# ssmiler/tfhe_fbs_map

Measured on AMD Instinct MI355X. Metric: functional bootstraps/sec (batched), N=1024, higher is better.
Workload: dtype f64 (exact integer arithmetic mod a 46-bit prime via FMA; residues in 64-bit words)

## Files before the change

### tfhe_fbs_map_amd/_native.py

```python
from __future__ import annotations

import ctypes as C
import operator
import os
import weakref

import numpy as np

_HERE = os.path.dirname(os.path.abspath(__file__))
LIB_PATH = os.environ.get("FBS_LIB") or os.path.join(_HERE, "libfbsexec.so")

from .security import MODULUS, MODULUS_BITS, sigma_min
from . import _client_native, _public_native
from ._client_native import GAUSSIAN_SAMPLER_GRADE, RANDOMNESS_GRADE, SAMPLERS, ClientContext, FbsError, Params, _Params, _c, _ptr, gpu_library_missing


class _Layout(C.Structure):
    _fields_ = [(f, C.c_uint32) for f in ("n_slots", "n_levels", "max_width", "max_sources", "n_bootstrap", "n_keyswitch",
                                          "n_inputs", "n_outputs", "n_rotations", "row_words")]


class _ProgramDesc(C.Structure):
    _fields_ = [("n_inputs", C.c_uint32), ("n_instr", C.c_uint32), ("n_terms", C.c_uint32),
                ("n_outputs", C.c_uint32),
# ... 751 lines not shown
        self._check(lib.fbs_refresh_compact_dev(self._h, d_words or None, count, self.default_compact_bits if bits is None else int(bits),
                                                d_cts or None, stream or None))

    def decrypt_compact_dev(self, d_words, count, d_msgs, bits=None, stream=0):
        self._check(lib.fbs_decrypt_compact_dev(self._h, d_words or None, count, self.default_compact_bits if bits is None else int(bits),
                                                d_msgs or None, stream or None))

    def _import_gadget_key(self, noun, t, gamma, bodies):
        bodies = _c(bodies, np.uint64).reshape(-1)
        if 1 <= int(t) <= 31 and bodies.size != self._gadget_key_sizes(noun, t)[0]:
            raise ValueError(f"{noun}_bodies has {bodies.size} words, the parameter set needs {self._gadget_key_sizes(noun, t)[0]}")
        self._check(getattr(lib, f"fbs_import_{noun}_key")(self._h, int(t), int(gamma), _ptr(bodies)))

    def import_packing_key(self, t_p, gamma_p, bodies):
        self._import_gadget_key("packing", t_p, gamma_p, bodies)

    def fold_keygen(self, t_f, gamma_f):
        self._check(lib.fbs_fold_keygen(self._h, int(t_f), int(gamma_f)))

    def fold_key_sizes(self, t_f=0):
        return self._gadget_key_sizes("fold", t_f)

    def export_fold_key(self, full=False):
        return self._export_gadget_key("fold", self.params.k * self.params.N, full)

    def import_fold_key(self, t_f, gamma_f, bodies):
        self._import_gadget_key("fold", t_f, gamma_f, bodies)

    def fold_dev(self, d_cts, count, d_glwe, stream=0):
        self._check(lib.fbs_fold_dev(self._h, d_cts or None, int(count), d_glwe or None, stream or None))

    def fold_mapped_dev(self, d_cts, n_src, d_map, count, d_glwe, stream=0):
        self._check(lib.fbs_fold_mapped_dev(self._h, d_cts or None, int(n_src), d_map or None, int(count), d_glwe or None, stream or None))

    def lookup_dev(self, d_tables, n_tables, d_table_of, d_cts_index, count, d_cts_out, stream=0):
        self._check(lib.fbs_lookup_dev(self._h, d_tables or None, int(n_tables), d_table_of or None, d_cts_index or None, int(count),
                                       d_cts_out or None, stream or None))

    def lookup_compact_dev(self, d_tables, n_tables, d_table_of, d_words, count, d_cts_out, bits=None, stream=0):
        self._check(lib.fbs_lookup_compact_dev(self._h, d_tables or None, int(n_tables), d_table_of or None, d_words or None, int(count),
                                               self.default_compact_bits if bits is None else int(bits), d_cts_out or None, stream or None))

    def rotate_dev(self, d_tables, n_tables, d_table_of, d_cts_index, count, d_glwe_out, negate=False, stream=0):
        self._check(lib.fbs_rotate_dev(self._h, d_tables or None, int(n_tables), d_table_of or None, d_cts_index or None, int(count),
                                       ROTATE_NEGATE if negate else 0, d_glwe_out or None, stream or None))

    def rotate_compact_dev(self, d_tables, n_tables, d_table_of, d_words, count, d_glwe_out, bits=None, negate=False, stream=0):
        self._check(lib.fbs_rotate_compact_dev(self._h, d_tables or None, int(n_tables), d_table_of or None, d_words or None, int(count),
                                               self.default_compact_bits if bits is None else int(bits), ROTATE_NEGATE if negate else 0,
                                               d_glwe_out or None, stream or None))

    def glwe_add_dev(self, d_dst, n_dst, dst_of, d_src, stream=0):
        dst_of = _c(dst_of, np.uint32).reshape(-1)
        self._check(lib.fbs_glwe_add_dev(self._h, d_dst or None, int(n_dst), _ptr(dst_of), d_src or None, dst_of.size, stream or None))

    def debug_fold_front_dev(self, d_cts, count, cols, tg, d_fields, stream=0):
        self._check(lib.fbs_debug_fold_front_dev(self._h, d_cts or None, int(count), int(cols), int(tg), d_fields or None, stream or None))

    def fold(self, cts):
        import torch
        cts = _c(cts, np.uint64).reshape(-1, self.params.ct_words)
        count, prm = cts.shape[0], self.params
        words = -(-count // prm.N) * (prm.k + 1) * prm.N
        dev = f"cuda:{self.device}"
        d_c = torch.from_numpy(cts.view(np.int64)).to(dev) if count else torch.zeros(1, dtype=torch.int64, device=dev)
        d_w = torch.zeros(max(2, words), dtype=torch.int64, device=dev)
        torch.cuda.synchronize(d_w.device)
        self.fold_dev(d_c.data_ptr(), count, d_w.data_ptr())
        self.sync()
        return d_w[:words].cpu().numpy().view(np.uint64)

    def pack_dev(self, d_cts, count, d_words, bits, stream=0):
        self._check(lib.fbs_pack_dev(self._h, d_cts or None, int(count), int(bits), d_words or None, stream or None))

    def debug_pack_fields_dev(self, d_fields, count, d_words, bits, stream=0):
        self._check(lib.fbs_debug_pack_fields_dev(self._h, d_fields or None, int(count), int(bits), d_words or None, stream or None))

    def pack(self, cts, bits):
        import torch
        cts = _c(cts, np.uint64).reshape(-1, self.params.ct_words)
        count = cts.shape[0]
        d_c = torch.from_numpy(cts.view(np.int64)).to("cuda:%d" % self.device)
        d_w = torch.zeros(max(1, self.packed_words(count, bits)), dtype=torch.int64, device=d_c.device)
        torch.cuda.synchronize(d_c.device)
        self.pack_dev(d_c.data_ptr(), count, d_w.data_ptr(), bits)
        self.sync()
        return d_w[:self.packed_words(count, bits)].cpu().numpy().view(np.uint64)

    def bootstrap_batch(self, tvset, cts, table_ids=None):
        cts = _c(cts, np.uint64)
        count = cts.size // self.params.ct_words
        ids = None if table_ids is None else _c(table_ids, np.uint32)
        out = np.empty_like(cts)
        self._check(lib.fbs_bootstrap_batch(self._h, tvset._h, _ptr(cts), _ptr(ids), count, _ptr(out)))
        return out

    def encrypt_dev(self, d_msgs, count, d_cts, nonce0=None, stream=0):
        if nonce0 is None:
            first = C.c_uint64()
            self._check(lib.fbs_encrypt_fresh_dev(self._h, d_msgs or None, count, d_cts or None, C.byref(first), stream or None))
            return first.value
        self._check(lib.fbs_encrypt_dev(self._h, d_msgs or None, count, int(nonce0), d_cts or None, stream or None))
        return int(nonce0)

    def decrypt_dev(self, d_cts, count, d_msgs, stream=0):
        self._check(lib.fbs_decrypt_dev(self._h, d_cts or None, count, d_msgs or None, stream or None))

    def bootstrap_batch_dev(self, tvset, d_in, d_table_ids, count, d_out, stream=0):
        self._check(lib.fbs_bootstrap_batch_dev(self._h, tvset._h, d_in, d_table_ids or None, count, d_out,
                                                stream or None))

    def lincomb_dev(self, d_wires, T, dst, term_off, srcs, coefs, consts, stream=0):
        dst, term_off, srcs = _c(dst, np.uint32), _c(term_off, np.uint32), _c(srcs, np.uint32)
        coefs, consts = _c(coefs, np.int64), _c(consts, np.int64)
        self._check(lib.fbs_lincomb_dev(self._h, d_wires, T, len(dst), _ptr(dst), _ptr(term_off), _ptr(srcs),
                                        _ptr(coefs), _ptr(consts), stream or None))

    def bootstrap_wires_dev(self, tvset, d_wires, T, src, dst, table_ids, s_begin, s_end, stream=0):
        src, dst, table_ids = _c(src, np.uint32), _c(dst, np.uint32), _c(table_ids, np.uint32)
        self._check(lib.fbs_bootstrap_wires_dev(self._h, tvset._h, d_wires, T, len(src), _ptr(src), _ptr(dst),
                                                _ptr(table_ids), s_begin, s_end, stream or None))

    def profile(self, on=True):
        self._check(lib.fbs_profile_enable(self._h, int(on)))

    def profile_read(self, reset=True):
        ms = (C.c_double * 3)()
        cnt = (C.c_uint64 * 3)()
        self._check(lib.fbs_profile_read(self._h, C.byref(ms), C.byref(cnt), int(reset)))
        names = ("keyswitch", "blind_rotate", "lincomb")
        return {n: dict(ms=ms[i], launches=int(cnt[i]), kernel=lib.fbs_profile_kernel(self._h, i).decode())
                for i, n in enumerate(names)}

    def profile_kernels(self):
        need = C.c_size_t()
        self._check(lib.fbs_profile_kernels(self._h, None, 0, C.byref(need)))
        buf = C.create_string_buffer(need.value)
        self._check(lib.fbs_profile_kernels(self._h, buf, need.value, None))
        out = {}
        for line in buf.value.decode().splitlines():
            kind, name, launches, ms = line.split("\t")
            out[name] = dict(kind=("keyswitch", "blind_rotate", "lincomb")[int(kind)], launches=int(launches), ms=float(ms))
        return out

    def sync(self, stream=0):
        self._check(lib.fbs_sync(self._h, stream or None))

    def debug_polymul(self, a, b):
        a, b = _c(a, np.uint64), _c(b, np.uint64)
        c = np.empty_like(a)
        self._check(lib.fbs_debug_polymul(self._h, _ptr(a), _ptr(b), _ptr(c)))
        return c

    DEBUG_FIELD_OPS = ("fp_mulmod", "fp_mulmod_exact", "fp_center", "fp_canon", "fp_canon_near", "fp_u64_round_trip")

    def debug_field(self, op, x, w=None):
        x = _c(x, np.int64)
        w = None if w is None else _c(w, np.int64)
        out = np.empty_like(x)
        self._check(lib.fbs_debug_field(self._h, self.DEBUG_FIELD_OPS.index(op), _ptr(x), _ptr(w), x.size, _ptr(out)))
        return out

    def debug_gauss_dev(self, words, sigma):
        import torch
        words = _c(words, np.uint64).reshape(-1, 6)
        dev = torch.device("cuda", self.device)
        d_words = torch.from_numpy(words.view(np.int64)).to(dev)
        d_out = torch.empty(words.shape[0], dtype=torch.int64, device=dev)
        self._check(lib.fbs_debug_gauss_dev(self._h, d_words.data_ptr(), words.shape[0], int(sigma), d_out.data_ptr(), None))
        self.sync()
        return d_out.cpu().numpy()

    def debug_transform(self, variant, values):
        values = _c(values, np.int64).reshape(-1, 1 << self.params.log_n_poly)
        out = np.empty_like(values)
        self._check(lib.fbs_debug_transform(self._h, variant.encode(), _ptr(values), _ptr(out), values.shape[0]))
        return out
```

### tfhe_fbs_map_amd/csrc/fbs_blind_rotate.hip

```cpp
#include <hip/hip_runtime.h>

#include <algorithm>
#include <type_traits>
#include <utility>

#include "fbs_blind_rotate.hpp"

namespace fbs {

template <int LOGN, int LL>
__global__ __launch_bounds__(1 << LL) void k_polymul(const uint64_t *a, const uint64_t *b, uint64_t *c, const double *tw_fwd,
                                                     const double *tw_inv, double n_inv) {
    using W = typename NttFor<LOGN, LL>::type;
    __shared__ double lds[2 * W::N];
    const uint32_t t = threadIdx.x;
    typename W::Xchg xc{lds, 0};
    double x[W::E], y[W::E];
#pragma unroll
    for (int m = 0; m < W::E; m++) {
        x[m] = fp_from_u64(a[W::template index_of<0>(t, m)]);
        y[m] = fp_from_u64(b[W::template index_of<0>(t, m)]);
    }
    W::forward(x, xc, t, Twiddles(tw_fwd + W::LANE_TABLE_OFFSET, tw_fwd));
    W::forward(y, xc, t, Twiddles(tw_fwd + W::LANE_TABLE_OFFSET, tw_fwd));
#pragma unroll
    for (int m = 0; m < W::E; m++) x[m] = fp_mulmod(fp_mulmod(x[m], fp_center(y[m])), n_inv);
    W::inverse(x, xc, t, Twiddles(tw_inv + W::LANE_TABLE_OFFSET, tw_inv));
#pragma unroll
    for (int m = 0; m < W::E; m++) c[W::template index_of<0>(t, m)] = fp_to_u64(fp_canon(x[m]));
}

template <int BYTES>
__device__ __forceinline__ void rotated_read(double &w, uint32_t from) {
    asm volatile("ds_read_b64 %0, %1 offset:%2" : "=v"(w) : "v"(from), "n"(BYTES) : "memory");
}
template <int C, int E, int LANES, int... M>
__device__ __forceinline__ void rotated_reads(double (&w)[E], uint32_t from, std::integer_sequence<int, M...>) {
    (rotated_read<((M + C) & (E - 1)) * LANES * 8>(w[M], from), ...);
}
template <int E, int LANES, int... C>
__device__ __forceinline__ void rotated_reads_for(uint32_t c, double (&w)[E], uint32_t from, std::integer_sequence<int, C...>) {
    ((c == (uint32_t)C ? rotated_reads<C, E, LANES>(w, from, std::make_integer_sequence<int, E>{}) : (void)0), ...);
}
template <int E>
__device__ __forceinline__ void rotated_reads_landed(double (&w)[E]) {
    asm volatile("s_waitcnt lgkmcnt(0)" ::: "memory");
#pragma unroll
    for (int m = 0; m < E; m++) asm volatile("" : "+v"(w[m]));
}

template <int LOGN, int LL, int DIG, int FPW, bool TURNS = true>
__global__ __launch_bounds__((2 << LL) * FPW) __attribute__((amdgpu_waves_per_eu(2))) void k_blind_rotate(BrArgs a) {
    using W = typename NttFor<LOGN, LL>::type;
    constexpr int FIRST = (DIG == 3 || DIG == 7) ? (has_fused_opening<W>::value ? 3 : 2) : (DIG == 2 || DIG == 6) ? 1 : 0;
    constexpr bool BOUNDED = DIG >= 1;
    constexpr bool ONE_LEVEL = DIG == 4, TWO_LEVELS = DIG >= 5;
#ifndef FBS_PEEL_MAX_LL
#define FBS_PEEL_MAX_LL 6
#endif
    constexpr bool PEEL = ONE_LEVEL || TWO_LEVELS || LL <= FBS_PEEL_MAX_LL;
    constexpr int N = W::N, E = W::E, LANES = W::LANES;
    constexpr bool PIECES = LL == 6;
    constexpr int GUARD = PIECES ? LANES : 0, REGION = GUARD + 2 * N;
    __shared__ double lds_all[FPW * 2 * REGION];
    const uint32_t sub = threadIdx.x >> (LL + 1);
    const uint32_t comp = __builtin_amdgcn_readfirstlane((threadIdx.x >> LL) & 1u);
    const uint32_t t = threadIdx.x & (LANES - 1);
    double *lds = lds_all + sub * (2 * REGION) + GUARD;
    double *mine = lds + comp * REGION;
    double *theirs = lds + (comp ^ 1u) * REGION;
    typename W::Xchg xc{mine, 0};
    Twiddles twf(a.tw_fwd + W::LANE_TABLE_OFFSET, a.tw_fwd), twi(a.tw_inv + W::LANE_TABLE_OFFSET, a.tw_inv);
    if constexpr (LL <= FBS_ONE_BUFFER_MAX_LL) {
        xc.stride = 0;
        double *table = mine + N;
        const double *src = (comp ? a.tw_inv : a.tw_fwd) + W::LANE_TABLE_OFFSET;
#pragma unroll
        for (int m = 0; m < E; m++) table[t + (uint32_t)LANES * m] = src[t + (uint32_t)LANES * m];
        __syncthreads();
        twf.lane = lds + N;
        twi.lane = lds + REGION + N;
    }

    const BrJob job = br_job<N>(a, (size_t)blockIdx.x * FPW + sub);
    const uint32_t *ms = job.ms;
    const uint32_t rows = 2 * a.l;
    double acc[E];
    br_acc_init<N, LANES, 2>(acc, a, job, t, comp != 0u ? 1u : 0u);
    const auto [round_scale, round_offset, sign_bits] = br_rounding(a.l, a.beta);

    const uint32_t t16 = t * 16u;
    uint32_t r_next = ms[0];
    constexpr int PRIO = !TURNS ? 0 : LL <= 6 ? FBS_PRIO_ONE_WAVE : FBS_PRIO_MULTI_WAVE;
    const uint32_t slot = PRIO ? wave_slot_parity() : 0u;
    for (uint32_t i = 0; i < a.n; i++) {
        lead_if<PRIO>(PRIO == 7 ? 2u * i : i, slot);
        const uint32_t r = __builtin_amdgcn_readfirstlane(r_next);
        r_next = ms[i + 1];
        if constexpr (FPW == 1)
            if (r == 0) continue;

        uint32_t digits[E];
        {
            double *buf = xc.next();
            if constexpr (LL <= FBS_ONE_BUFFER_MAX_LL) W::sync();
#pragma unroll
            for (int m = 0; m < E; m++) buf[t + (uint32_t)LANES * m] = acc[m];
            if constexpr (PIECES) {
                constexpr int LOGE = LOGN - LL;
                buf[(int)t - LANES] = -acc[E - 1];
                W::sync();
                const uint32_t first = (0u - (r >> LL)) & (uint32_t)(2 * E - 1);
                const uint32_t from = (uint32_t)(uintptr_t)buf + 8u * (t - (r & (uint32_t)(LANES - 1)));
                double w[E];
                rotated_reads_for<E, LANES>(first & (uint32_t)(E - 1), w, from, std::make_integer_sequence<int, E>{});
                rotated_reads_landed(w);
#pragma unroll
                for (int m = 0; m < E; m++) {
                    const double sign = __hiloint2double((int)(0x3FF00000u | (((first + (uint32_t)m) << (31 - LOGE)) & 0x80000000u)), 0);
                    const double d = __builtin_fma(w[m], sign, -acc[m]);
                    digits[m] = (uint32_t)__builtin_fma(d, round_scale, round_offset) ^ sign_bits;
                }
            } else {
                W::sync();
                const uint32_t from = (t - r) & (2u * N - 1u);
#pragma unroll
                for (int m = 0; m < E; m++) {
                    const uint32_t idx = from + (uint32_t)LANES * m;
                    const double w = buf[idx & (N - 1)];
                    const double v = __hiloint2double(__double2hiint(w) ^ (int)((idx << (31 - LOGN)) & 0x80000000u), __double2loint(w));
                    const double d = v - acc[m];
                    digits[m] = (uint32_t)__builtin_fma(d, round_scale, round_offset) ^ sign_bits;
                }
            }
        }

        double own[E], other[E];
        auto level = [&](int lv, auto assign) {
            constexpr bool ASSIGN = decltype(assign)::value;
            const uint32_t shift = ((uint32_t)a.l - 1u - (uint32_t)lv) * a.beta;
            double x[E];
#pragma unroll
            for (int m = 0; m < E; m++)
                x[m] = (double)(int)__builtin_amdgcn_sbfe(digits[m], shift, a.beta);
            const KeyRows keys(a.bsk_hat + (size_t)FBS_KEY_STEP(i) * rows * 2 * N);
            const uint32_t krow = ((comp * a.l + (uint32_t)lv) * 2u) * (uint32_t)(N * 8);
            const uint32_t k_own = krow + comp * (uint32_t)(N * 8), k_oth = krow + (comp ^ 1u) * (uint32_t)(N * 8);
            constexpr int EARLY = E / 4;
            double2 ko[E / 2];
            W::template forward<FIRST>(x, xc, t, twf, [&] {
#pragma unroll
                for (int m = 0; m < EARLY; m++) ko[m] = keys.load(t16 + (uint32_t)(m * LANES * 16), k_own);
            });
#pragma unroll
            for (int m = EARLY; m < E / 2; m++) ko[m] = keys.load(t16 + (uint32_t)(m * LANES * 16), k_own);
            double2 kt[E / 2];
#pragma unroll
            for (int j = 0; j < E / 2; j++) {
                const double p0 = fp_mulmod(x[2 * j], ko[j].x), p1 = fp_mulmod(x[2 * j + 1], ko[j].y);
                own[2 * j] = ASSIGN ? p0 : own[2 * j] + p0;
                own[2 * j + 1] = ASSIGN ? p1 : own[2 * j + 1] + p1;
                kt[j] = keys.load(t16 + (uint32_t)(j * LANES * 16), k_oth);
            }
#pragma unroll
            for (int j = 0; j < E / 2; j++) {
                const double p0 = fp_mulmod(x[2 * j], kt[j].x), p1 = fp_mulmod(x[2 * j + 1], kt[j].y);
                other[2 * j] = ASSIGN ? p0 : other[2 * j] + p0;
                other[2 * j + 1] = ASSIGN ? p1 : other[2 * j + 1] + p1;
            }
        };
        if constexpr (TWO_LEVELS) {
            level(1, std::true_type{});
            level(0, std::false_type{});
        } else if constexpr (PEEL) {
            level((int)a.l - 1, std::true_type{});
            if constexpr (!ONE_LEVEL)
                for (int lv = (int)a.l - 2; lv >= 0; lv--) level(lv, std::false_type{});
        } else {
#pragma unroll
            for (int m = 0; m < E; m++) own[m] = other[m] = 0.0;
            for (int lv = (int)a.l - 1; lv >= 0; lv--) level(lv, std::false_type{});
        }

        const typename W::InvUniform inv_uni = W::inverse_uniform(t, twi);
        {
            const uint32_t slot = xc.pp ? xc.stride : 0;
            xc.pp ^= 1u;
            if constexpr (LL <= FBS_ONE_BUFFER_MAX_LL) __syncthreads();
#pragma unroll
            for (int m = 0; m < E; m++) theirs[slot + W::handoff_word(t, m)] = other[m];
            __syncthreads();
#pragma unroll
            for (int m = 0; m < E; m++) own[m] += mine[slot + W::handoff_word(t, m)];
        }

        if constexpr (PRIO == 7) lead_if<PRIO>(2u * i + 1u, slot);
        if constexpr (has_fused_opening<W>::value && BOUNDED)
            W::inverse_exit_centred(own, xc, t, twi, inv_uni);
        else
            W::template inverse<BOUNDED>(own, xc, t, twi, inv_uni);
#pragma unroll
        for (int m = 0; m < E; m++) acc[m] = fp_center(acc[m] + own[m]);
    }

    if constexpr (FPW == 4) {
        if (!job.live) return;
        if (uint64_t *raw = gate_acc(a.gv, job.f, 2 * N)) {
#pragma unroll
            for (int m = 0; m < E; m++) raw[comp * N + t + (uint32_t)LANES * m] = fp_to_u64(fp_canon(acc[m]));
            return;
        }
        uint64_t *out = gate_out(a.gv, job.f, a.ct_words);
        if (comp == 0) {
#pragma unroll
            for (int m = 0; m < E; m++) {
                const uint32_t j = t + (uint32_t)LANES * m;
                const uint64_t v = fp_to_u64(fp_canon(acc[m]));
                if (j == 0) out[0] = v;
                else out[N - j] = fq_neg(v);
            }
        } else if (t == 0) {
            const uint64_t b = fp_to_u64(fp_canon(acc[0]));
            out[N] = a.post ? fq_add(b, a.post[job.table]) : b;
        }
    } else {
        br_extract<N, LANES, 2>(a, job, acc, comp, t);
    }
}

template <int LOGN, int LL, int DIG>
__global__ __launch_bounds__(2 << LL) __attribute__((amdgpu_waves_per_eu(2))) void k_blind_rotate_pairs(BrArgs a) {
    using W = typename NttFor<LOGN, LL>::type;
    static_assert(W::HAS_EVAL_POSITION, "the bundle needs to know which evaluation point a register holds");
    constexpr int N = W::N, E = W::E, LANES = W::LANES;
    constexpr int FIRST = DIG == 3 ? 2 : 0;
    constexpr bool ONE_LEVEL = DIG == 4;
    __shared__ __attribute__((aligned(16384))) double lds_all[2 * 2 * N + N];
    constexpr int GLOG = W::EVAL_GROUP_LOG2, G = 1 << GLOG;
    const uint32_t comp = __builtin_amdgcn_readfirstlane((threadIdx.x >> LL) & 1u);
    const uint32_t t = threadIdx.x & (LANES - 1);
    double *lds = lds_all;
    double *mine = lds + comp * 2 * N;
    double *theirs = lds + (comp ^ 1u) * 2 * N;
    typename W::Xchg xc{mine, 0};
    Twiddles twf(a.tw_fwd + W::LANE_TABLE_OFFSET, a.tw_fwd), twi(a.tw_inv + W::LANE_TABLE_OFFSET, a.tw_inv);
    static_assert(LL <= FBS_ONE_BUFFER_MAX_LL, "one exchange buffer per polynomial, twiddle tables beside it");
    {
        xc.stride = 0;
        double *table = mine + N;
        const double *src = (comp ? a.tw_inv : a.tw_fwd) + W::LANE_TABLE_OFFSET;
#pragma unroll
        for (int m = 0; m < E; m++) table[t + (uint32_t)LANES * m] = src[t + (uint32_t)LANES * m];
#pragma unroll
        for (int m = 0; m < E / 2; m++) {
            const uint32_t x = comp * (N / 2) + t + (uint32_t)LANES * m;
            lds[4 * N + (x & (G - 1)) * (N / G) + (x >> GLOG)] = a.psi_pow[x];
        }
        __syncthreads();
        twf.lane = lds + N;
        twi.lane = lds + 3 * N;
    }

    const BrJob job = br_job<N>(a, blockIdx.x);
    const uint32_t *ms = job.ms;
    const uint32_t rows = 2 * a.l;
    double acc[E];
    br_acc_init<N, LANES, 2>(acc, a, job, t, comp != 0u ? 1u : 0u);
    const auto [round_scale, round_offset, sign_bits] = br_rounding(a.l, a.beta);
    const uint32_t o_lane = 2u * (__builtin_bitreverse32(W::eval_position_lane(t)) >> (32 - LOGN)) + 1u;
    const uint32_t k_lane8 = (o_lane >> GLOG) << 3;
    const uint32_t r_lane = __builtin_amdgcn_readfirstlane(o_lane & (G - 1));
    constexpr uint32_t MASK8 = (uint32_t)(N / G - 1) << 3;
    const uint32_t psi_base = (uint32_t)(uintptr_t)(lds + 4 * N);

    const uint32_t t16 = t * 16u;
    const uint32_t n_pairs = a.n / 2;
    uint32_t e0_next = ms[0], e1_next = ms[1];
    constexpr int PRIO = LL <= 6 ? FBS_PRIO_ONE_WAVE : FBS_PRIO_MULTI_WAVE;
    const uint32_t slot = PRIO ? wave_slot_parity() : 0u;
    for (uint32_t i = 0; i < n_pairs; i++) {
        lead_if<PRIO>(PRIO == 7 ? 2u * i : i, slot);
        uint32_t e[3];
        e[0] = __builtin_amdgcn_readfirstlane(e0_next);
        e[1] = __builtin_amdgcn_readfirstlane(e1_next);
        e0_next = ms[2 * i + 2 < a.n ? 2 * i + 2 : a.n];
        e1_next = ms[2 * i + 3 < a.n ? 2 * i + 3 : a.n];
        if (e[0] == 0 && e[1] == 0) continue;
        e[2] = (e[0] + e[1]) & (2u * N - 1u);
        uint32_t lane8[3];
#pragma unroll
        for (int jj = 0; jj < 3; jj++) lane8[jj] = __umul24(e[jj], k_lane8);

        uint32_t digits[E];
#pragma unroll
        for (int m = 0; m < E; m++) digits[m] = (uint32_t)__builtin_fma(acc[m], round_scale, round_offset) ^ sign_bits;

        double own[E], other[E];
        auto level = [&](int lv, auto assign) {
            constexpr bool ASSIGN = decltype(assign)::value;
            const uint32_t shift = ((uint32_t)a.l - 1u - (uint32_t)lv) * a.beta;
            double x[E];
#pragma unroll
            for (int m = 0; m < E; m++) x[m] = (double)(int)__builtin_amdgcn_sbfe(digits[m], shift, a.beta);
            uint32_t e_lv[3] = {e[0], e[1], e[2]};
            if constexpr (!ONE_LEVEL) asm volatile("" : "+s"(e_lv[0]), "+s"(e_lv[1]), "+s"(e_lv[2]));
            const KeyRows keys(a.bsk_hat + (size_t)FBS_KEY_STEP(i) * 3 * rows * 2 * N);
            uint32_t k_own[3], k_oth[3];
#pragma unroll
            for (int jj = 0; jj < 3; jj++) {
                const uint32_t krow = (((uint32_t)jj * rows + comp * a.l + (uint32_t)lv) * 2u) * (uint32_t)(N * 8);
                k_own[jj] = krow + comp * (uint32_t)(N * 8);
                k_oth[jj] = krow + (comp ^ 1u) * (uint32_t)(N * 8);
            }
            struct PairKeys {
                double2 ko[3], kt[3];
            };
            auto request = [&](auto jc, PairKeys &in) {
                constexpr int j = decltype(jc)::value;
#pragma unroll
                for (int jj = 0; jj < 3; jj++) {
                    in.ko[jj] = keys.load(t16 + (uint32_t)(j * LANES * 16), k_own[jj]);
                    in.kt[jj] = keys.load(t16 + (uint32_t)(j * LANES * 16), k_oth[jj]);
                }
            };
// ... 37 lines not shown
                own[2 * j + 1] = ASSIGN ? p1 : own[2 * j + 1] + p1;
                other[2 * j] = ASSIGN ? r0 : other[2 * j] + r0;
                other[2 * j + 1] = ASSIGN ? r1 : other[2 * j + 1] + r1;
            };
            PairKeys in;
            W::template forward<FIRST>(x, xc, t, twf, [&] { request(std::integral_constant<int, 0>{}, in); });
            static_assert(E == 16, "eight register pairs, written out");
#define FBS_PAIR_STEP(J)                                                                                    \
    if constexpr ((J) > 0) request(std::integral_constant<int, (J)>{}, in);                                 \
    consume(std::integral_constant<int, (J)>{}, in);                                                        \
    if constexpr (!ONE_LEVEL) __builtin_amdgcn_sched_barrier(0);
            FBS_PAIR_STEP(0) FBS_PAIR_STEP(1) FBS_PAIR_STEP(2) FBS_PAIR_STEP(3)
            FBS_PAIR_STEP(4) FBS_PAIR_STEP(5) FBS_PAIR_STEP(6) FBS_PAIR_STEP(7)
#undef FBS_PAIR_STEP
        };
        level((int)a.l - 1, std::true_type{});
        if constexpr (!ONE_LEVEL)
            for (int lv = (int)a.l - 2; lv >= 0; lv--) level(lv, std::false_type{});

        const typename W::InvUniform inv_uni = W::inverse_uniform(t, twi);
        {
            __syncthreads();
#pragma unroll
            for (int m = 0; m < E; m++) theirs[W::handoff_word(t, m)] = other[m];
            __syncthreads();
#pragma unroll
            for (int m = 0; m < E; m++) own[m] += mine[W::handoff_word(t, m)];
        }
        if constexpr (PRIO == 7) lead_if<PRIO>(2u * i + 1u, slot);
        W::template inverse<true>(own, xc, t, twi, inv_uni);
#pragma unroll
        for (int m = 0; m < E; m++) acc[m] = fp_center(acc[m] + own[m]);
    }

    br_extract<N, LANES, 2>(a, job, acc, comp, t);
}

#define FBS_FOR_EACH_SHAPE(X) X(8) X(9) X(10) X(11) X(12)

template <int LOGN>
static int transform_bsk_t(fbs_ctx *ctx, const uint64_t *d_given) {
    constexpr int LL = lanes_log2_for(LOGN);
    const fbs_params &p = ctx->p;
    const uint32_t N = ctx->N;
    const size_t polys = ctx->n_ggsw * ctx->rows * (p.k + 1);
    uint64_t *d_own = nullptr;
    hipError_t e = hipSuccess;
    if (!d_given) {
        FBS_HIP(ctx, hipMalloc(&d_own, polys * N * 8));
        e = hipMemcpyAsync(d_own, ctx->bsk.data(), polys * N * 8, hipMemcpyHostToDevice, ctx->stream);
        ctx->bsk_upload_bytes = (int64_t)(polys * N * 8);
    }
    const uint64_t *d_src = d_given ? d_given : d_own;
    if (e == hipSuccess) {
        const double n_inv = fq_centered(fq_inv(N));
        unsigned grid = (unsigned)std::min<size_t>(polys, 4096);
        hipLaunchKernelGGL((k_key_transform<LOGN, LL, KeyWords>), dim3(grid), dim3(1 << LL), 0, ctx->stream, KeyWords{d_src},
                           reinterpret_cast<double *>(ctx->d_bsk_hat), reinterpret_cast<const double *>(ctx->d_tw_fwd), n_inv,
                           polys);
        e = hipGetLastError();
        constexpr int LLS = lanes_log2_for_small_launch(LOGN);
        if (small_key_needed(ctx)) {
            if (e == hipSuccess && !ctx->d_bsk_hat_small) e = hipMalloc(&ctx->d_bsk_hat_small, polys * N * 8);
            if (e == hipSuccess) {
                hipLaunchKernelGGL((k_key_transform<LOGN, LLS, KeyWords>), dim3(grid), dim3(1 << LLS), 0, ctx->stream, KeyWords{d_src},
                                   reinterpret_cast<double *>(ctx->d_bsk_hat_small), reinterpret_cast<const double *>(ctx->d_tw_fwd),
                                   n_inv, polys);
                e = hipGetLastError();
            }
        }
    }
    if (e == hipSuccess) e = hipStreamSynchronize(ctx->stream);
    if (d_own) (void)hipFree(d_own);
    if (e != hipSuccess) return set_error(ctx, FBS_E_DEVICE, std::string("bootstrapping-key transform: ") + hipGetErrorString(e));
    return FBS_OK;
}

int dev_transform_bsk(fbs_ctx *ctx, const uint64_t *d_src) {
    switch (ctx->p.log_n_poly) {
#define X(L) case L: return transform_bsk_t<L>(ctx, d_src);
        FBS_FOR_EACH_SHAPE(X)
#undef X
    }
    return set_error(ctx, FBS_E_INVALID, "unsupported N");
}

int dev_upload_tables(fbs_ctx *ctx) {
    const fbs_params &p = ctx->p;
    const uint32_t N = ctx->N;
    std::vector<uint64_t> fwd, inv;
    host_twiddles(p.log_n_poly, fwd, inv);
    std::vector<double> fwd_c(tw_table_words(N)), inv_c(tw_table_words(N));
    for (uint32_t i = 0; i < tw_table_words(N); i++) {
        fwd_c[i] = fq_centered(fwd[i]);
        inv_c[i] = fq_centered(inv[i]);
    }
    const size_t bsk_words = ctx->n_ggsw * ctx->rows * (p.k + 1) * N;
    const size_t ksk_rows = (size_t)ctx->D * p.t_ksk;
    if (!ctx->d_tw_fwd) {
        FBS_HIP(ctx, hipMalloc(&ctx->d_tw_fwd, (size_t)tw_table_words(N) * 8));
        FBS_HIP(ctx, hipMalloc(&ctx->d_tw_inv, (size_t)tw_table_words(N) * 8));
        FBS_HIP(ctx, hipMalloc(&ctx->d_bsk_hat, bsk_words * 8));
        FBS_HIP(ctx, hipMalloc(&ctx->d_ksk, ksk_rows * ctx->ksk_stride * 8));
        FBS_HIP(ctx, hipMalloc(&ctx->d_ksk_f, ksk_rows * ctx->ksk_stride * 8));
        FBS_HIP(ctx, hipMalloc(&ctx->d_ks_corr, (size_t)ctx->ksk_stride * 8));
    }
    FBS_HIP(ctx, hipMemcpyAsync(ctx->d_tw_fwd, fwd_c.data(), fwd_c.size() * 8, hipMemcpyHostToDevice, ctx->stream));
    FBS_HIP(ctx, hipMemcpyAsync(ctx->d_tw_inv, inv_c.data(), inv_c.size() * 8, hipMemcpyHostToDevice, ctx->stream));
    if (ctx->group == 2) {
        std::vector<double> tbl(N);
        const uint64_t psi = fq_pow(FQ_GENERATOR, (FQ - 1) / (2ull * N));
        uint64_t pw = 1;
        for (uint32_t x = 0; x < N; x++) {
            tbl[x] = fq_centered(pw);
            pw = fq_mul(pw, psi);
        }
        if (!ctx->d_psi_pow) FBS_HIP(ctx, hipMalloc(&ctx->d_psi_pow, tbl.size() * 8));
        FBS_HIP(ctx, hipMemcpy(ctx->d_psi_pow, tbl.data(), tbl.size() * 8, hipMemcpyHostToDevice));
    }
    FBS_HIP(ctx, hipStreamSynchronize(ctx->stream));
    return FBS_OK;
}

int dev_upload_ksk(fbs_ctx *ctx) {
    const fbs_params &p = ctx->p;
    const size_t ksk_rows = (size_t)ctx->D * p.t_ksk;
    std::vector<uint64_t> corr(ctx->ksk_stride, 0);
    {
        std::vector<unsigned __int128> sum(p.n + 1, 0);
        for (size_t r = 0; r < ksk_rows; r++)
            for (uint32_t i = 0; i <= p.n; i++) sum[i] += ctx->ksk[r * (p.n + 1) + i];
        for (uint32_t i = 0; i <= p.n; i++) corr[i] = fq_mul((uint64_t)(sum[i] % FQ), 1ull << (p.gamma_ksk - 1));
    }
    FBS_HIP(ctx, hipMemcpyAsync(ctx->d_ks_corr, corr.data(), corr.size() * 8, hipMemcpyHostToDevice, ctx->stream));
    FBS_HIP(ctx, hipMemsetAsync(ctx->d_ksk, 0, ksk_rows * ctx->ksk_stride * 8, ctx->stream));
    FBS_HIP(ctx, hipMemcpy2DAsync(ctx->d_ksk, (size_t)ctx->ksk_stride * 8, ctx->ksk.data(), (size_t)(p.n + 1) * 8,
                                  (size_t)(p.n + 1) * 8, ksk_rows, hipMemcpyHostToDevice, ctx->stream));
    {
        std::vector<double> kf(ksk_rows * (size_t)ctx->ksk_stride, 0.0);
        for (size_t r = 0; r < ksk_rows; r++)
            for (uint32_t i = 0; i <= p.n; i++) kf[r * ctx->ksk_stride + i] = fq_centered(ctx->ksk[r * (p.n + 1) + i]);
        FBS_HIP(ctx, hipMemcpy(ctx->d_ksk_f, kf.data(), kf.size() * 8, hipMemcpyHostToDevice));
    }
    FBS_HIP(ctx, hipStreamSynchronize(ctx->stream));
    return dev_keyswitch_gemm_setup(ctx);
}

int dev_upload_keys(fbs_ctx *ctx) {
    if (int rc = dev_upload_tables(ctx)) return rc;
    if (int rc = dev_upload_ksk(ctx)) return rc;
    return dev_transform_bsk(ctx, nullptr);
}

static bool launch_blind_rotate_main(const Kernel &k, const BrArgs &a, hipStream_t stream) {
    if (k.family == Family::BLIND_ROTATE) {
#define X(L, LL, DIG, FPW, TURNS)                                                                                               \
    if (k.t[0] == L && k.t[1] == (LL) && k.t[2] == DIG && k.t[3] == FPW && k.alt == !(TURNS)) {                                 \
        hipLaunchKernelGGL((k_blind_rotate<L, LL, DIG, FPW, TURNS>), dim3((unsigned)((a.count + FPW - 1) / FPW)),              \
                           dim3((2 << (LL)) * FPW), 0, stream, a);                                                              \
        return true;                                                                                                            \
    }
        FBS_BR_KERNELS(X)
#undef X
    }
    if (k.family == Family::PAIRS) {
#define X(L, DIG)                                                                                                               \
    if (k.t[0] == L && k.t[1] == lanes_log2_for(L) && k.t[2] == DIG) {                                                          \
        hipLaunchKernelGGL((k_blind_rotate_pairs<L, lanes_log2_for(L), DIG>), dim3((unsigned)a.count), dim3(2 << lanes_log2_for(L)), \
                           0, stream, a);                                                                                       \
        return true;                                                                                                            \
    }
        FBS_PAIRS_KERNELS(X)
#undef X
    }
    return false;
}

int dev_blind_rotate(fbs_ctx *ctx, const fbs_tvset *tv, const GateView &gv, const uint32_t *d_ms, hipStream_t stream,
                     const BrStart *start) {
    const fbs_params &p = ctx->p;
    BrArgs a{};
    if (start) {
        if (start->whole) {
            if (gv.acc_rows || !gv.out_rows || !gv.dst_slot || gv.row_words != (p.k + 1) * ctx->N)
                return set_error(ctx, FBS_E_INVALID, "a rotated sample goes into rows of (k + 1) N words");
        } else if (gv.acc_rows || gv.row_words) {
            return set_error(ctx, FBS_E_INVALID, "a rotation of an encrypted table cannot be a fused one");
        }
        if (!start->d_acc0 || start->n_acc == 0) return set_error(ctx, FBS_E_INVALID, "no encrypted table to rotate");
        a.acc0 = start->d_acc0;
        a.n_acc = start->n_acc;
        a.acc_of = start->d_acc_of;
    } else if (!tv) {
        return set_error(ctx, FBS_E_INVALID, "null argument");
    }
    a.ms = d_ms;
    a.tw_fwd = reinterpret_cast<const double *>(ctx->d_tw_fwd);
    a.tw_inv = reinterpret_cast<const double *>(ctx->d_tw_inv);
    a.psi_pow = reinterpret_cast<const double *>(ctx->d_psi_pow);
    a.tvs = tv ? tv->d_tvs : nullptr;
    a.post = tv && !start ? tv->d_post : nullptr;
    a.n = p.n;
    a.l = p.l_bsk;
    a.beta = p.beta_bsk;
    a.ct_words = ctx->D + 1;
    a.n_tables = !tv ? 1u : (gv.acc_rows || gv.row_words) ? tv->n_tables + 1 : std::max(1u, tv->n_tables);
    if (gv.count > 0x7FFFFFFFull) return set_error(ctx, FBS_E_INVALID, "batch too large for one launch");
    for (const Launch &l : select_blind_rotate(ctx, gv.count)) {
        a.gv = gv;
        a.gv.f_begin += l.first;
        a.gv.count = a.count = l.count;
        a.acc_first = (uint32_t)((start ? start->first : 0) + l.first);
        if (a.gv.out_rows) a.gv.out_rows += l.first * (size_t)(gv.row_words ? gv.row_words : ctx->D + 1);
        a.bsk_hat = reinterpret_cast<const double *>(reads_small_key(l.kernel) ? ctx->d_bsk_hat_small : ctx->d_bsk_hat);
        ctx->prof.kernel[1] = kernel_name(l.kernel);
        hipEvent_t e0, e1;
        prof_begin(ctx, 1, stream, &e0, &e1);
        if (!launch_blind_rotate_main(l.kernel, a, stream) && !launch_blind_rotate_cu(l.kernel, a, stream) &&
            !launch_blind_rotate_k2(l.kernel, a, stream) && !launch_blind_rotate_glwe(l.kernel, a, stream)) {
            if (e0) ctx->prof.pool.push_back({e0, e1});
            return set_error(ctx, FBS_E_INVALID, "no instantiation of " + ctx->prof.kernel[1]);
        }
        prof_end(ctx, 1, stream, e0, e1);
        FBS_HIP(ctx, hipGetLastError());
    }
    return FBS_OK;
}

int dev_polymul(fbs_ctx *ctx, const uint64_t *d_a, const uint64_t *d_b, uint64_t *d_c, hipStream_t stream) {
    const double n_inv = fq_centered(fq_inv(ctx->N));
    const double *twf = reinterpret_cast<const double *>(ctx->d_tw_fwd), *twi = reinterpret_cast<const double *>(ctx->d_tw_inv);
    switch (ctx->p.log_n_poly) {
#define X(L)                                                                                                               \
    case L:                                                                                                                \
        hipLaunchKernelGGL((k_polymul<L, lanes_log2_for(L)>), dim3(1), dim3(1 << lanes_log2_for(L)), 0, stream, d_a, d_b, \
                           d_c, twf, twi, n_inv);                                                                          \
        break;
        FBS_FOR_EACH_SHAPE(X)
#undef X
        default: return set_error(ctx, FBS_E_INVALID, "unsupported N");
    }
    FBS_HIP(ctx, hipGetLastError());
    return FBS_OK;
}

}
```

### tfhe_fbs_map_amd/csrc/fbs_debug_transform.hip

```cpp
#include <hip/hip_runtime.h>

#include <cstdio>
#include <cstring>
#include <string>
#include <type_traits>
#include <vector>

#include "fbs_blind_rotate_cu.hpp"

namespace fbs {

__global__ void k_debug_field(int op, const long long *x, const long long *w, size_t count, long long *out) {
    const size_t i = (size_t)blockIdx.x * blockDim.x + threadIdx.x;
    if (i >= count) return;
    const double a = (double)x[i], b = w ? (double)w[i] : 0.0;
    long long r = 0;
    switch (op) {
    case 0: r = (long long)fp_mulmod(a, b); break;
    case 1: r = (long long)fp_mulmod_exact(a, b); break;
    case 2: r = (long long)fp_center(a); break;
    case 3: r = (long long)fp_canon(a); break;
    case 4: r = (long long)fp_canon_near(a); break;
    case 5: r = (long long)fp_to_u64(fp_from_u64((uint64_t)x[i])); break;
    }
    out[i] = r;
}

int dev_debug_field(fbs_ctx *ctx, int op, const int64_t *x, const int64_t *w, size_t count, int64_t *out) {
    if (op < 0 || op > 5 || !x || !out || (op <= 1 && !w)) return set_error(ctx, FBS_E_INVALID, "debug_field: bad operation or null array");
    if (count == 0) return FBS_OK;
    if (count > (1u << 26)) return set_error(ctx, FBS_E_INVALID, "debug_field: too many operands");
    const size_t bytes = count * 8;
    long long *d = nullptr;
    FBS_HIP(ctx, hipMalloc(&d, 3 * bytes));
    hipError_t e = hipMemcpy(d, x, bytes, hipMemcpyHostToDevice);
    if (e == hipSuccess && w) e = hipMemcpy(d + count, w, bytes, hipMemcpyHostToDevice);
    if (e == hipSuccess) {
        hipLaunchKernelGGL(k_debug_field, dim3((unsigned)((count + 255) / 256)), dim3(256), 0, ctx->stream, op, d, w ? d + count : nullptr, count,
                           d + 2 * count);
        e = hipGetLastError();
    }
    if (e == hipSuccess) e = hipStreamSynchronize(ctx->stream);
    if (e == hipSuccess) e = hipMemcpy(out, d + 2 * count, bytes, hipMemcpyDeviceToHost);
    (void)hipFree(d);
    if (e != hipSuccess) return set_error(ctx, FBS_E_DEVICE, std::string("debug_field: ") + hipGetErrorString(e));
    return FBS_OK;
}

template <class W>
__device__ __forceinline__ Twiddles debug_twiddles(double *lds, const double *tw, uint32_t t) {
    static_assert(W::LANES <= (1 << FBS_ONE_BUFFER_MAX_LL), "every shape exchanges through one buffer");
#pragma unroll
    for (int m = 0; m < W::E; m++) lds[W::N + t + (uint32_t)W::LANES * m] = tw[W::LANE_TABLE_OFFSET + t + (uint32_t)W::LANES * m];
    __syncthreads();
    return Twiddles(lds + W::N, tw);
}

template <class W, int FIRST>
__global__ __launch_bounds__(W::LANES) void k_debug_forward(const long long *in, long long *out, const double *tw_fwd, const double *) {
    __shared__ double lds[2 * W::N];
    const uint32_t t = threadIdx.x;
    const Twiddles twf = debug_twiddles<W>(lds, tw_fwd, t);
    typename W::Xchg xc{lds, 0};
    xc.stride = 0;
    const long long *src = in + (size_t)blockIdx.x * W::N;
    long long *dst = out + (size_t)blockIdx.x * W::N;
    double x[W::E];
#pragma unroll
    for (int m = 0; m < W::E; m++) x[m] = (double)src[W::template index_of<0>(t, m)];
    W::template forward<FIRST>(x, xc, t, twf, typename W::NoHook{});
#pragma unroll
    for (int m = 0; m < W::E; m++) dst[t * W::E + m] = (long long)x[m];
}

template <class W, bool BOUNDED>
__global__ __launch_bounds__(W::LANES) void k_debug_inverse(const long long *in, long long *out, const double *, const double *tw_inv) {
    __shared__ double lds[2 * W::N];
    const uint32_t t = threadIdx.x;
    const Twiddles twi = debug_twiddles<W>(lds, tw_inv, t);
    typename W::Xchg xc{lds, 0};
    xc.stride = 0;
    const long long *src = in + (size_t)blockIdx.x * W::N;
    long long *dst = out + (size_t)blockIdx.x * W::N;
    double x[W::E];
#pragma unroll
    for (int m = 0; m < W::E; m++) x[m] = (double)src[t * W::E + m];
    const typename W::InvUniform inv_uni = W::inverse_uniform(t, twi);
    W::template inverse<BOUNDED>(x, xc, t, twi, inv_uni);
#pragma unroll
    for (int m = 0; m < W::E; m++) dst[W::template index_of<0>(t, m)] = (long long)x[m];
}

template <class W>
__global__ __launch_bounds__(W::LANES) void k_debug_inverse_exit_centred(const long long *in, long long *out, const double *, const double *tw_inv) {
    __shared__ double lds[2 * W::N];
    const uint32_t t = threadIdx.x;
    const Twiddles twi = debug_twiddles<W>(lds, tw_inv, t);
    typename W::Xchg xc{lds, 0};
    xc.stride = 0;
    const long long *src = in + (size_t)blockIdx.x * W::N;
    long long *dst = out + (size_t)blockIdx.x * W::N;
    double x[W::E];
#pragma unroll
    for (int m = 0; m < W::E; m++) x[m] = (double)src[t * W::E + m];
    const typename W::InvUniform inv_uni = W::inverse_uniform(t, twi);
    W::inverse_exit_centred(x, xc, t, twi, inv_uni);
#pragma unroll
    for (int m = 0; m < W::E; m++) dst[W::template index_of<0>(t, m)] = (long long)x[m];
}

template <int LOGN, int NP>
__global__ __launch_bounds__(256) void k_debug_lane_forward(const long long *in, long long *out, const double *tw_fwd, const double *tw_inv) {
    using W = WavesNtt<LOGN, 2>;
    using Part = typename W::Half;
    constexpr int N = W::N, E = W::E, M = W::M;
    __shared__ double lds[NP * N + CuTwiddles<Part, false>::LDS_WORDS];
    const uint32_t t = threadIdx.x, w = W::wave_of(t), ln = t & 63u;
    CuTwiddles<Part, false> tw;
    tw.init((uniform_doubles)(uintptr_t)tw_fwd, (uniform_doubles)(uintptr_t)tw_inv, tw_fwd + W::LANE_TABLE_OFFSET, tw_inv + W::LANE_TABLE_OFFSET, w,
            ln, lds + NP * N);
    __syncthreads();
    const size_t base = (size_t)blockIdx.x * NP * N;
    double x[NP][E];
    double *bufs[NP];
#pragma unroll
    for (int p = 0; p < NP; p++) {
        bufs[p] = lds + p * N + w * M;
#pragma unroll
        for (int m = 0; m < E; m++) x[p][m] = (double)in[base + (size_t)p * N + w * M + ln + 64u * m];
    }
    tw.template forward<NP>(x, bufs, ln);
#pragma unroll
    for (int p = 0; p < NP; p++)
#pragma unroll
        for (int m = 0; m < E; m++) out[base + (size_t)p * N + t * E + m] = (long long)x[p][m];
}

template <int LOGN>
__global__ __launch_bounds__(256) void k_debug_lane_inverse(const long long *in, long long *out, const double *tw_fwd, const double *tw_inv) {
    using W = WavesNtt<LOGN, 2>;
    using Part = typename W::Half;
    constexpr int N = W::N, E = W::E, M = W::M;
    __shared__ double lds[N + CuTwiddles<Part, false>::LDS_WORDS];
    const uint32_t t = threadIdx.x, w = W::wave_of(t), ln = t & 63u;
    CuTwiddles<Part, false> tw;
    tw.init((uniform_doubles)(uintptr_t)tw_fwd, (uniform_doubles)(uintptr_t)tw_inv, tw_fwd + W::LANE_TABLE_OFFSET, tw_inv + W::LANE_TABLE_OFFSET, w,
            ln, lds + N);
    __syncthreads();
    const size_t base = (size_t)blockIdx.x * N;
    double x[E];
#pragma unroll
    for (int m = 0; m < E; m++) x[m] = (double)in[base + t * E + m];
    tw.inverse(x, lds + w * M, ln, typename Part::NoHook{});
#pragma unroll
    for (int m = 0; m < E; m++) out[base + w * M + ln + 64u * m] = (long long)x[m];
}

template <class W>
constexpr int br_first(int dig) {
    return (dig == 3 || dig == 7) ? (has_fused_opening<W>::value ? 3 : 2) : (dig == 2 || dig == 6) ? 1 : 0;
}
constexpr bool br_bounded(int dig) { return dig >= 1; }
constexpr int pairs_first(int dig) { return dig == 3 ? 2 : 0; }

template <class W>
struct NttClass;
template <int LOGN, int LL>
struct NttClass<PolyNtt<LOGN, LL>> {
    static constexpr const char *name = "PolyNtt";
    static constexpr int logn = LOGN;
};
template <int LOGN, int LL>
struct NttClass<SplitNtt<LOGN, LL>> {
    static constexpr const char *name = "SplitNtt";
    static constexpr int logn = LOGN;
};
template <int LOGN, int LOGW>
struct NttClass<WavesNtt<LOGN, LOGW>> {
    static constexpr const char *name = "WavesNtt";
    static constexpr int logn = LOGN;
};
template <class Part>
constexpr const char *lane_class() {
    return std::is_same<Part, LaneNtt256>::value ? "LaneNtt256" : "LaneNtt512";
}

typedef void (*DebugKernel)(const long long *, long long *, const double *, const double *);
struct Variant {
    std::string line;
    int logn, lanes, np;
    DebugKernel kernel;
    bool listed = true;
};

static void add(std::vector<Variant> &v, const char *cls, int logn, int lanes, const char *dir, const char *what, int value, int np,
                DebugKernel kernel) {
// ... 95 lines not shown
```

### tfhe_fbs_map_amd/csrc/fbs_field.hpp

```cpp
#pragma once
#include <stdint.h>

#if defined(__HIPCC__)
#define FBS_HD __host__ __device__ __forceinline__
#define FBS_D __device__ __forceinline__
#else
#define FBS_HD inline
#endif

namespace fbs {

constexpr uint64_t FQ = 0x3FFFFFF84001ull;
constexpr int FQ_BITS = 46;
constexpr uint64_t FQ_GENERATOR = 7;

FBS_HD uint64_t fq_add(uint64_t a, uint64_t b) {
    uint64_t s = a + b;
    return s >= FQ ? s - FQ : s;
}
FBS_HD uint64_t fq_sub(uint64_t a, uint64_t b) { return a >= b ? a - b : a + FQ - b; }
FBS_HD uint64_t fq_neg(uint64_t a) { return a ? FQ - a : 0; }
FBS_HD uint64_t fq_mul(uint64_t a, uint64_t b) { return (uint64_t)(((unsigned __int128)a * b) % FQ); }
FBS_HD uint64_t fq_from_i64(int64_t v) {
    if (v >= 0) return (uint64_t)v % FQ;
    uint64_t m = (0 - (uint64_t)v) % FQ;
    return m ? FQ - m : 0;
}
FBS_HD uint64_t fq_fold(uint64_t r) {
    r >>= 64 - FQ_BITS;
    return r >= FQ ? r - FQ : r;
}
inline uint64_t fq_pow(uint64_t a, uint64_t e) {
    uint64_t r = 1;
    while (e) {
        if (e & 1) r = fq_mul(r, a);
        a = fq_mul(a, a);
        e >>= 1;
    }
    return r;
}
inline uint64_t fq_inv(uint64_t a) { return fq_pow(a, FQ - 2); }
inline double fq_centered(uint64_t a) { return a > FQ / 2 ? -(double)(FQ - a) : (double)a; }

constexpr uint32_t tw_fused_word(uint32_t n) { return 3 * n; }
constexpr uint32_t tw_table_words(uint32_t n) { return 3 * n + 2; }

#if defined(__HIPCC__)
constexpr double FP_Q = 70368743669761.0;
constexpr double FP_QINV = 1.0 / 70368743669761.0;
constexpr double FP_MAGIC = 4503599627370496.0;

FBS_D double fp_mulmod(double x, double w) {
    const double h = x * w;
    const double l = __builtin_fma(x, w, -h);
    const double qh = __builtin_rint(h * FP_QINV);
    return __builtin_fma(-qh, FP_Q, h) + l;
}
FBS_D double fp_mulmod_exact(double x, double w) {
    const double h = x * w;
    return __builtin_fma(-__builtin_rint(h * FP_QINV), FP_Q, h);
}
FBS_D double fp_center(double x) { return __builtin_fma(-__builtin_rint(x * FP_QINV), FP_Q, x); }
FBS_D double fp_canon(double x) {
    const double c = fp_center(x);
    return c < 0.0 ? c + FP_Q : c;
}
FBS_D double fp_canon_near(double x) { return __builtin_fma(-__builtin_floor(x * FP_QINV), FP_Q, x); }
#define FBS_CHECK_MULTIPLE(k) static_assert(((k) * FP_Q) * FP_QINV == (k), "k*q/q must be exact")
FBS_CHECK_MULTIPLE(1.0); FBS_CHECK_MULTIPLE(2.0); FBS_CHECK_MULTIPLE(3.0); FBS_CHECK_MULTIPLE(4.0);
FBS_CHECK_MULTIPLE(5.0); FBS_CHECK_MULTIPLE(6.0); FBS_CHECK_MULTIPLE(7.0); FBS_CHECK_MULTIPLE(8.0);
FBS_CHECK_MULTIPLE(9.0); FBS_CHECK_MULTIPLE(10.0); FBS_CHECK_MULTIPLE(11.0); FBS_CHECK_MULTIPLE(12.0);
#undef FBS_CHECK_MULTIPLE
FBS_D double fp_exp2i(int e) { return __longlong_as_double((long long)(1023 + e) << 52); }
FBS_D uint64_t fp_to_u64(double x) { return (uint64_t)__double_as_longlong(x + FP_MAGIC) & 0x000FFFFFFFFFFFFFull; }
FBS_D double fp_from_u64(uint64_t v) {
    return __longlong_as_double((long long)(v | 0x4330000000000000ull)) - FP_MAGIC;
}
#endif

}
```

Baseline: 112,200.

## Fuse three-level key products into one modular reduction in blind rotate

Adds a SUM3 variant of the blind-rotate kernel for N=1024, LL=6, DIG=3 with three decomposition levels. It forward-transforms all three digit polynomials first, then accumulates the three key products with a magic-constant FMA summation and a single modular reduction per output. Key loads are double-buffered and interleaved with the products. The aim is fewer reductions, fewer separate key-load passes and better load/compute overlap, at the cost of more live registers for three digit arrays and exactness that rests on operand ranges.

```diff
diff --git a/tfhe_fbs_map_amd/_native.py b/tfhe_fbs_map_amd/_native.py
--- a/tfhe_fbs_map_amd/_native.py
+++ b/tfhe_fbs_map_amd/_native.py
@@ -927,13 +927,18 @@
         self._check(lib.fbs_debug_polymul(self._h, _ptr(a), _ptr(b), _ptr(c)))
         return c
 
-    DEBUG_FIELD_OPS = ("fp_mulmod", "fp_mulmod_exact", "fp_center", "fp_canon", "fp_canon_near", "fp_u64_round_trip")
+    DEBUG_FIELD_OPS = ("fp_mulmod", "fp_mulmod_exact", "fp_center", "fp_canon", "fp_canon_near", "fp_u64_round_trip", "fp_sum3_mulmod")
 
     def debug_field(self, op, x, w=None):
         x = _c(x, np.int64)
         w = None if w is None else _c(w, np.int64)
-        out = np.empty_like(x)
-        self._check(lib.fbs_debug_field(self._h, self.DEBUG_FIELD_OPS.index(op), _ptr(x), _ptr(w), x.size, _ptr(out)))
+        if op == "fp_sum3_mulmod":
+            if w is None or x.ndim != 2 or x.shape[1] != 3 or w.shape != x.shape:
+                raise ValueError("fp_sum3_mulmod takes two [count][3] arrays")
+            out = np.empty(x.shape[0], dtype=np.int64)
+        else:
+            out = np.empty_like(x)
+        self._check(lib.fbs_debug_field(self._h, self.DEBUG_FIELD_OPS.index(op), _ptr(x), _ptr(w), out.size, _ptr(out)))
         return out
 
     def debug_gauss_dev(self, words, sigma):
diff --git a/tfhe_fbs_map_amd/csrc/fbs_blind_rotate.hip b/tfhe_fbs_map_amd/csrc/fbs_blind_rotate.hip
--- a/tfhe_fbs_map_amd/csrc/fbs_blind_rotate.hip
+++ b/tfhe_fbs_map_amd/csrc/fbs_blind_rotate.hip
@@ -49,8 +49,9 @@
     for (int m = 0; m < E; m++) asm volatile("" : "+v"(w[m]));
 }
 
-template <int LOGN, int LL, int DIG, int FPW, bool TURNS = true>
+template <int LOGN, int LL, int DIG, int FPW, bool TURNS = true, bool SUM3 = false>
 __global__ __launch_bounds__((2 << LL) * FPW) __attribute__((amdgpu_waves_per_eu(2))) void k_blind_rotate(BrArgs a) {
+    static_assert(!SUM3 || (DIG == 3 && LL == 6 && LOGN == 10), "the summed products rest on the ranges of the fused opening");
     using W = typename NttFor<LOGN, LL>::type;
     constexpr int FIRST = (DIG == 3 || DIG == 7) ? (has_fused_opening<W>::value ? 3 : 2) : (DIG == 2 || DIG == 6) ? 1 : 0;
     constexpr bool BOUNDED = DIG >= 1;
@@ -169,7 +170,50 @@
                 other[2 * j + 1] = ASSIGN ? p1 : other[2 * j + 1] + p1;
             }
         };
-        if constexpr (TWO_LEVELS) {
+        if constexpr (SUM3) {
+            const KeyRows keys(a.bsk_hat + (size_t)FBS_KEY_STEP(i) * 6 * 2 * N);
+            const uint32_t krow = comp * (uint32_t)(3 * 2 * N * 8);
+            const uint32_t k_own = krow + comp * (uint32_t)(N * 8), k_oth = krow + (comp ^ 1u) * (uint32_t)(N * 8);
+            constexpr uint32_t LEVEL = 2 * N * 8;
+            struct PairKeys {
+                double2 ko[3], kt[3];
+            };
+            auto request = [&](int j, PairKeys &in) {
+#pragma unroll
+                for (int lv = 0; lv < 3; lv++) {
+                    in.ko[lv] = keys.load(t16 + (uint32_t)((j & 3) * LANES * 16), k_own + (uint32_t)lv * LEVEL + (uint32_t)((j >> 2) * 4 * LANES * 16));
+                    in.kt[lv] = keys.load(t16 + (uint32_t)((j & 3) * LANES * 16), k_oth + (uint32_t)lv * LEVEL + (uint32_t)((j >> 2) * 4 * LANES * 16));
+                }
+            };
+            auto digits_of = [&](double (&x)[E], uint32_t shift) {
+#pragma unroll
+                for (int m = 0; m < E; m++) x[m] = (double)(int)__builtin_amdgcn_sbfe(digits[m], shift, a.beta);
+            };
+            double x2[E], x1[E], x0[E];
+            PairKeys in[2];
+            digits_of(x2, 0u);
+            W::template forward<FIRST>(x2, xc, t, twf, typename W::NoHook{});
+            __builtin_amdgcn_sched_barrier(0);
+            digits_of(x1, a.beta);
+            W::template forward<FIRST>(x1, xc, t, twf, typename W::NoHook{});
+            __builtin_amdgcn_sched_barrier(0);
+            digits_of(x0, 2u * a.beta);
+            W::template forward<FIRST>(x0, xc, t, twf, [&] { request(0, in[0]); });
+            __builtin_amdgcn_sched_barrier(0);
+#pragma unroll
+            for (int j = 0; j < E / 2; j++) {
+                if (j + 1 < E / 2) request(j + 1, in[(j + 1) & 1]);
+                const PairKeys &k = in[j & 1];
+                own[2 * j] = fp_sum3_mulmod(x2[2 * j], k.ko[2].x, x1[2 * j], k.ko[1].x, x0[2 * j], k.ko[0].x);
+                own[2 * j + 1] = fp_sum3_mulmod(x2[2 * j + 1], k.ko[2].y, x1[2 * j + 1], k.ko[1].y, x0[2 * j + 1], k.ko[0].y);
+                asm volatile("" : "+v"(own[2 * j]), "+v"(own[2 * j + 1]));
+                __builtin_amdgcn_sched_barrier(0);
+                other[2 * j] = fp_sum3_mulmod(x2[2 * j], k.kt[2].x, x1[2 * j], k.kt[1].x, x0[2 * j], k.kt[0].x);
+                other[2 * j + 1] = fp_sum3_mulmod(x2[2 * j + 1], k.kt[2].y, x1[2 * j + 1], k.kt[1].y, x0[2 * j + 1], k.kt[0].y);
+                asm volatile("" : "+v"(other[2 * j]), "+v"(other[2 * j + 1]));
+                __builtin_amdgcn_sched_barrier(0);
+            }
+        } else if constexpr (TWO_LEVELS) {
             level(1, std::true_type{});
             level(0, std::false_type{});
         } else if constexpr (PEEL) {
@@ -513,10 +557,19 @@
     return dev_transform_bsk(ctx, nullptr);
 }
 
+constexpr bool br_sum3_built(int logn, int ll, int dig, int fpw, bool turns) { return logn == 10 && ll == 6 && dig == 3 && (fpw == 4 || fpw == 1) && turns; }
+
 static bool launch_blind_rotate_main(const Kernel &k, const BrArgs &a, hipStream_t stream) {
     if (k.family == Family::BLIND_ROTATE) {
 #define X(L, LL, DIG, FPW, TURNS)                                                                                               \
     if (k.t[0] == L && k.t[1] == (LL) && k.t[2] == DIG && k.t[3] == FPW && k.alt == !(TURNS)) {                                 \
+        if constexpr (br_sum3_built(L, LL, DIG, FPW, TURNS)) {                                                                  \
+            if (a.l == 3) {                                                                                                     \
+                hipLaunchKernelGGL((k_blind_rotate<L, LL, DIG, FPW, TURNS, br_sum3_built(L, LL, DIG, FPW, TURNS)>),             \
+                                   dim3((unsigned)((a.count + FPW - 1) / FPW)), dim3((2 << (LL)) * FPW), 0, stream, a);         \
+                return true;                                                                                                    \
+            }                                                                                                                   \
+        }                                                                                                                       \
         hipLaunchKernelGGL((k_blind_rotate<L, LL, DIG, FPW, TURNS>), dim3((unsigned)((a.count + FPW - 1) / FPW)),              \
                            dim3((2 << (LL)) * FPW), 0, stream, a);                                                              \
         return true;                                                                                                            \
diff --git a/tfhe_fbs_map_amd/csrc/fbs_debug_transform.hip b/tfhe_fbs_map_amd/csrc/fbs_debug_transform.hip
--- a/tfhe_fbs_map_amd/csrc/fbs_debug_transform.hip
+++ b/tfhe_fbs_map_amd/csrc/fbs_debug_transform.hip
@@ -13,6 +13,11 @@
 __global__ void k_debug_field(int op, const long long *x, const long long *w, size_t count, long long *out) {
     const size_t i = (size_t)blockIdx.x * blockDim.x + threadIdx.x;
     if (i >= count) return;
+    if (op == 6) {
+        out[i] = (long long)fp_sum3_mulmod((double)x[3 * i], (double)w[3 * i], (double)x[3 * i + 1], (double)w[3 * i + 1], (double)x[3 * i + 2],
+                                           (double)w[3 * i + 2]);
+        return;
+    }
     const double a = (double)x[i], b = w ? (double)w[i] : 0.0;
     long long r = 0;
     switch (op) {
@@ -27,21 +32,23 @@
 }
 
 int dev_debug_field(fbs_ctx *ctx, int op, const int64_t *x, const int64_t *w, size_t count, int64_t *out) {
-    if (op < 0 || op > 5 || !x || !out || (op <= 1 && !w)) return set_error(ctx, FBS_E_INVALID, "debug_field: bad operation or null array");
+    const bool two = op <= 1 || op == 6;
+    if (op < 0 || op > 6 || !x || !out || (two && !w)) return set_error(ctx, FBS_E_INVALID, "debug_field: bad operation or null array");
     if (count == 0) return FBS_OK;
     if (count > (1u << 26)) return set_error(ctx, FBS_E_INVALID, "debug_field: too many operands");
+    const size_t in = (op == 6 ? 3 : 1) * count;
     const size_t bytes = count * 8;
     long long *d = nullptr;
-    FBS_HIP(ctx, hipMalloc(&d, 3 * bytes));
-    hipError_t e = hipMemcpy(d, x, bytes, hipMemcpyHostToDevice);
-    if (e == hipSuccess && w) e = hipMemcpy(d + count, w, bytes, hipMemcpyHostToDevice);
+    FBS_HIP(ctx, hipMalloc(&d, (2 * in + count) * 8));
+    hipError_t e = hipMemcpy(d, x, in * 8, hipMemcpyHostToDevice);
+    if (e == hipSuccess && w) e = hipMemcpy(d + in, w, in * 8, hipMemcpyHostToDevice);
     if (e == hipSuccess) {
-        hipLaunchKernelGGL(k_debug_field, dim3((unsigned)((count + 255) / 256)), dim3(256), 0, ctx->stream, op, d, w ? d + count : nullptr, count,
-                           d + 2 * count);
+        hipLaunchKernelGGL(k_debug_field, dim3((unsigned)((count + 255) / 256)), dim3(256), 0, ctx->stream, op, d, w ? d + in : nullptr, count,
+                           d + 2 * in);
         e = hipGetLastError();
     }
     if (e == hipSuccess) e = hipStreamSynchronize(ctx->stream);
-    if (e == hipSuccess) e = hipMemcpy(out, d + 2 * count, bytes, hipMemcpyDeviceToHost);
+    if (e == hipSuccess) e = hipMemcpy(out, d + 2 * in, bytes, hipMemcpyDeviceToHost);
     (void)hipFree(d);
     if (e != hipSuccess) return set_error(ctx, FBS_E_DEVICE, std::string("debug_field: ") + hipGetErrorString(e));
     return FBS_OK;
diff --git a/tfhe_fbs_map_amd/csrc/fbs_field.hpp b/tfhe_fbs_map_amd/csrc/fbs_field.hpp
--- a/tfhe_fbs_map_amd/csrc/fbs_field.hpp
+++ b/tfhe_fbs_map_amd/csrc/fbs_field.hpp
@@ -56,6 +56,16 @@
     const double qh = __builtin_rint(h * FP_QINV);
     return __builtin_fma(-qh, FP_Q, h) + l;
 }
+constexpr double FP_SUM3_BIG = 3802951800684688204490109616128.0;
+static_assert(FP_SUM3_BIG == 1.5 * 2535301200456458802993406410752.0, "1.5 * 2^101");
+FBS_D double fp_sum3_mulmod(double x2, double k2, double x1, double k1, double x0, double k0) {
+    const double a0 = __builtin_fma(x2, k2, FP_SUM3_BIG), g0 = a0 - FP_SUM3_BIG, l0 = __builtin_fma(x2, k2, -g0);
+    const double a1 = __builtin_fma(x1, k1, a0), g1 = a1 - a0, l1 = __builtin_fma(x1, k1, -g1);
+    const double a2 = __builtin_fma(x0, k0, a1), g2 = a2 - a1, l2 = __builtin_fma(x0, k0, -g2);
+    const double h = a2 - FP_SUM3_BIG, l = (l0 + l1) + l2;
+    const double qh = __builtin_rint((h + l) * FP_QINV);
+    return __builtin_fma(-qh, FP_Q, h) + l;
+}
 FBS_D double fp_mulmod_exact(double x, double w) {
     const double h = x * w;
     return __builtin_fma(-__builtin_rint(h * FP_QINV), FP_Q, h);
```

Measured after the change: 112,100. About the same (-0.1%).
